# davidepi/glaze

Measured on AMD Instinct MI355X. Metric: Msamples/s + achieved HBM GB/s, Sponza 1080p, 1/2/4/8xMI355X, higher is better.
Workload: dtype f32; 1 GPU; Sponza-class synthetic atrium (262267 tris, 26 materials, 27 textures) as a .glaze V1 file (2853389 bytes) through parse, 1920x1080, path tracer depth 8, 143 steps = 17.9 spp; materials=26, textures=27, scene=Sponza-class synthetic atrium, width=1920, height=1080, depth=8, triangles=262267

## Files before the change

glaze_amd/csrc/abi.cpp:

```cpp
#include <cstring>
#include <string>
#include <vector>

#include "abi_internal.h"
#include "serializer.h"
#include "converter.h"
#include "codec/jpeg.h"
#include "codec/png_enc.h"
#include <strings.h>
#include "rccl_dl.h"

using namespace glz;
using namespace glz::abi;

namespace {
thread_local std::string g_error;
thread_local int g_status = GLZ_OK;

template <class T>
int64_t copy_out(const std::vector<T>& v, T* out, int64_t cap) {
  if (out && cap > 0) memcpy(out, v.data(), sizeof(T) * (size_t)std::min<int64_t>(cap, (int64_t)v.size()));
  return (int64_t)v.size();
}
}
// ... 265 lines not shown
  Renderer* r = Renderer::create(inst->i.get(), scene ? scene->s : std::shared_ptr<Scene>(), w, h, e);
  if (!r) {
    fail(e);
    return nullptr;
  }
  glz_renderer* hr = new glz_renderer();
  hr->r.reset(r);
  return hr;
  GLZ_GUARD_END(nullptr)
}
void glz_renderer_destroy(glz_renderer* h) { delete h; }



int glz_renderer_set_integrator(glz_renderer* h, int i) { GLZ_GUARD_BEGIN GLZ_R(h); GLZ_RET(h->r->set_integrator(i, e)); GLZ_GUARD_END(GLZ_E_IO) }
int glz_renderer_set_exposure(glz_renderer* h, float x) { GLZ_GUARD_BEGIN GLZ_R(h); GLZ_RET(h->r->set_exposure(x)); GLZ_GUARD_END(GLZ_E_IO) }
int glz_renderer_update_camera(glz_renderer* h, const glz_camera* c) {
  GLZ_GUARD_BEGIN GLZ_R(h);
  if (!c) return fail(GLZ_E_ARG, "camera is null");
  GLZ_RET(h->r->update_camera(*c, e));
  GLZ_GUARD_END(GLZ_E_IO)
}
int glz_renderer_change_resolution(glz_renderer* h, uint32_t w, uint32_t hh) { GLZ_GUARD_BEGIN GLZ_R(h); GLZ_RET(h->r->change_resolution(w, hh, e)); GLZ_GUARD_END(GLZ_E_IO) }
int glz_renderer_change_scene(glz_renderer* h, glz_scene* s) {
  GLZ_GUARD_BEGIN GLZ_R(h);
  if (!s || !s->s || !s->owned) return fail(GLZ_E_ARG, "scene is null or already owned by a renderer");
  s->owned = false;
  GLZ_RET(h->r->change_scene(s->s, e));
  GLZ_GUARD_END(GLZ_E_IO)
}
int glz_renderer_update_materials_and_lights(glz_renderer* h, const glz_material* m, uint32_t nm, const glz_light* l, uint32_t nl,
// ... 190 lines not shown
```

glaze_amd/csrc/device/path_state.h:

```cpp
#pragma once
#include <hip/hip_runtime.h>

#include "device/intersect.h"
#include "device/math.h"
#include "device/trace_wave.h"
#include "kernels.h"

namespace glz {
using namespace dev;

constexpr uint32_t kQueueShards = 8;
constexpr uint32_t kCounterStride = 32;
constexpr uint32_t kFlagUpdate = 1u;
constexpr uint32_t kFlagShadow = 2u;

struct PixelId {
  uint32_t x, y;
  bool active;
};
__device__ __forceinline__ PixelId pixel_of(const TileMap& m, uint32_t lid) {
  const uint32_t lane = lid & 63u, sub = (lid >> 6) & 63u, ltile = lid >> 12;
  const uint32_t gtile = ltile * m.world + m.rank;
  const uint32_t tx = gtile % m.tiles_x, ty = gtile / m.tiles_x;
  PixelId p;
// ... 42 lines not shown
      origin = mk3(ro.x, ro.y, ro.z);
      direction = mk3(rd.x, rd.y, rd.z);
    }
    tmin = 0.0001f;
    tmax = INFINITY;
    return true;
  }
};
struct ClosestSink {
  const LaunchArgs& A;
  __device__ __forceinline__ void store(uint32_t lid, const HitRecord& h) {
    A.st.hit[lid] = make_float4(h.leaf == 0xFFFFFFFFu ? INFINITY : h.t, h.u, h.v, __uint_as_float(h.leaf));
  }
};

__device__ __forceinline__ void accumulate_pixel(const LaunchArgs& A, uint32_t lid, vec3 c, bool add, bool update, float exposure, float4 cum) {
  cum.w += 1.0f;
  if (update) {
    if (add) { cum.x += c.x; cum.y += c.y; cum.z += c.z; }
    A.st.result[lid] = make_float4(cum.x * exposure / cum.w, cum.y * exposure / cum.w, cum.z * exposure / cum.w, 1.0f);
  }
  A.st.cumulative[lid] = cum;
}
__device__ __forceinline__ void accumulate_pixel(const LaunchArgs& A, uint32_t lid, vec3 c, bool add, bool update, float exposure) {
  accumulate_pixel(A, lid, c, add, update, exposure, A.st.cumulative[lid]);
}

__device__ __forceinline__ uint32_t queue_capacity(uint32_t n_local_pixels) {
  const uint32_t blocks = (n_local_pixels + kBlock - 1) / kBlock;
  return ((blocks + kQueueShards - 1) / kQueueShards) * kBlock;
}
__device__ __forceinline__ uint32_t queue_slot(uint32_t* counters, uint32_t n_local_pixels, bool push) {
  const unsigned long long m = __ballot(push);
  uint32_t slot = 0;
  if (push) {
    const uint32_t shard = ((blockIdx.x * blockDim.x + threadIdx.x) / kBlock) % kQueueShards;
    const int lane = threadIdx.x & 63;
    const int leader = __ffsll((long long)m) - 1;
    uint32_t base = 0;
    if (lane == leader) base = atomicAdd(counters + shard * kCounterStride, (uint32_t)__popcll(m));
// ... 18 lines not shown
    contrib = A.st.contrib[q];
    lid = __float_as_uint(sd.w);
    o = mk3(so.x, so.y, so.z);
    d = mk3(sd.x, sd.y, sd.z);
    tmin = 0.001f;
    tmax = so.w;
    return true;
  }
};
struct ShadowSink {
  const LaunchArgs& A;
  ShadowSource& src;
  __device__ __forceinline__ void store(uint32_t, const HitRecord& h) {
    const bool occluded = h.leaf != 0xFFFFFFFFu;
    const vec3 c = mk3(src.contrib.x, src.contrib.y, src.contrib.z);
    const bool add = !occluded;
    accumulate_pixel(A, src.lid, c, add, true, A.shadow_exposure);
  }
};
}
```

glaze_amd/csrc/device/shade_pixel.h:

```cpp
#pragma once
#include <hip/hip_runtime.h>

#include "device/hit_vertex.h"
#include "device/math.h"
#include "device/path_state.h"
#include "device/shading.h"
#include "device/types.h"
#include "kernels.h"

namespace glz {
using namespace dev;

struct SharedQueue {
  const LaunchArgs& A;
  __device__ __forceinline__ uint32_t slot(bool push) { return queue_slot(A.st.queue_count + A.shade_set * kQueueSetWords, A.map.n_local_pixels, push); }
};
#ifdef GLZ_SECTION_TIMES
#define GLZ_SHADE_STAMP(k) out.stamp(k)
#else
#define GLZ_SHADE_STAMP(k) do { } while (0)
#endif
struct DirectState {
  const LaunchArgs& A;
  __device__ __forceinline__ void stamp(int) {}
  __device__ __forceinline__ void ray_o(uint32_t lid, float4 v) { A.st.ray_o[lid] = v; }
  __device__ __forceinline__ void ray_d(uint32_t lid, float4 v) { A.st.ray_d[lid] = v; }
  __device__ __forceinline__ void imp(int q, uint32_t lid, float4 v) { A.st.imp[q][lid] = v; }
  __device__ __forceinline__ float4 read_imp(int q, uint32_t lid) const { return A.st.imp[q][lid]; }
  __device__ __forceinline__ void accumulate(uint32_t lid, vec3 c, bool add, bool update, float exposure) { accumulate_pixel(A, lid, c, add && isfinite(c.x + c.y + c.z), update, exposure); }
};
struct StagedState {
#ifdef GLZ_SECTION_TIMES
  unsigned long long sec[8] = {0, 0, 0, 0, 0, 0, 0, 0}, sec_last = 0;
  __device__ __forceinline__ void stamp(int k) {
    const unsigned long long now = __builtin_amdgcn_s_memtime();
    sec[k] += now - sec_last;
    sec_last = now;
  }
#else
  __device__ __forceinline__ void stamp(int) {}
#endif
  float4 ro, rd, im[4];
  uint32_t mask = 0;
  __device__ __forceinline__ void ray_o(uint32_t, float4 v) { ro = v; mask |= 1u; }
  __device__ __forceinline__ void ray_d(uint32_t, float4 v) { rd = v; mask |= 2u; }
  __device__ __forceinline__ void imp(int q, uint32_t, float4 v) { im[q] = v; mask |= 4u; }
  const LaunchArgs* A = nullptr;
  LdsNodePtr lds_imp = nullptr;
  static constexpr uint32_t kShadeBlockPixels = 256;
  __device__ __forceinline__ float4 read_imp(int q, uint32_t) const {
    const u32x4 v = lds_imp[q * kShadeBlockPixels];
    return make_float4(__uint_as_float(v.x), __uint_as_float(v.y), __uint_as_float(v.z), __uint_as_float(v.w));
  }
  __device__ __forceinline__ void accumulate(uint32_t lid, vec3 cc, bool add, bool update, float exposure) { accumulate_pixel(*A, lid, cc, add && isfinite(cc.x + cc.y + cc.z), update, exposure); }
};
template <bool LOD, class Queue, class State>
__device__ __forceinline__ int shade_pixel_body(const LaunchArgs& A, const DeviceScene& S, const FrameData& F, uint32_t lid, PixelId px, float4 ro, float4 rd, float4 hr, Queue& queue,
                                                State& out, float& end_w) {
  const bool fresh = F.direct_only || ro.w == 0.0f;
  float bounce = F.direct_only ? 0.0f : ro.w;
  const vec3 direction = mk3(rd.x, rd.y, rd.z);
  auto load_importance = [&]() {
    asm volatile("" ::: "memory");
    Spec imp;
    if (fresh) {
      imp = spec_set(1.0f);
    } else {
#pragma unroll
      for (int q = 0; q < 4; ++q) {
// ... 2 lines not shown
      }
    }
    return imp;
  };
  const uint32_t leaf = __float_as_uint(hr.w);
  if (leaf == 0xFFFFFFFFu) {
    uint32_t flags = 0;
    vec3 c = mk3(0.0f, 0.0f, 0.0f);
    if ((bounce == 0.0f || rd.w == 1.0f) && S.sky.tex_id > 0) {
      const vec3 w = normalize3(xform_dir(S.sky.world2obj, direction));
      const float phi = glz_atan2f(w.y, w.x), theta = glz_acosf(w.z);
      const vec3 texel = texture_rgb(S, S.sky.tex_id, vec2{phi * kInv2Pi, theta * kInvPi});
      c = spec_to_rgb(spec_mul(load_importance(), from_illuminant_color(texel)));
      flags = kFlagUpdate;
    }
    out.accumulate(lid, c, true, flags != 0, F.exposure);
    end_w = rd.w;
    return F.direct_only ? 0 : 1;
  }
  HitVertex hv = load_hit_vertex(S, hr, [&]() { return A.st.hit_inst[lid]; });
  const MatScalars mat = hv.mat;
  GLZ_SHADE_STAMP(0);
  TexFootprint fp{kNoLod, 0.0f, 0.0f, 1u};
  float cone_w = 0.0f;
  if constexpr (LOD) {
    const auto& [va0, va1, vb0, vb1, vc0, vc1, dn, du_rec] = hv.rec;
    float cone_in = F.cone_width0;
    asm volatile("" : "+v"(cone_in));
    if (!fresh) cone_in = A.st.cone[lid];
    cone_w = cone_in + F.cone_spread * hr.x;
    vec3 e1 = mk3(vb0.x, vb0.y, vb0.z) - mk3(va0.x, va0.y, va0.z), e2 = mk3(vc0.x, vc0.y, vc0.z) - mk3(va0.x, va0.y, va0.z);
// ... 79 lines not shown
      }
    }
    if (!(flags & kFlagShadow)) {
      const Spec importance = load_importance();
      imp_lum = spec_luminance(importance);
      have_lum = true;
    }
    const bool push = (flags & kFlagShadow) != 0;
    GLZ_SHADE_STAMP(3);
    const uint32_t slot = queue.slot(push);
    if (push) {
      A.st.sh_o[slot] = make_float4(point.x, point.y, point.z, sh_tmax);
      A.st.sh_d[slot] = make_float4(sh_dir.x, sh_dir.y, sh_dir.z, __uint_as_float(lid));
      A.st.contrib[slot] = make_float4(c.x, c.y, c.z, __uint_as_float(flags));
    } else {
      out.accumulate(lid, c, true, true, F.exposure);
    }
    spec_flag = 0.0f;
  } else {
    out.accumulate(lid, mk3(0.0f, 0.0f, 0.0f), false, false, F.exposure);
    spec_flag = 1.0f;
  }
  if (F.direct_only) return 0;
  GLZ_SHADE_STAMP(4);
  float rr_scale = 1.0f;
  if (bounce > (float)(F.pt_steps / 2u)) {
    const float kill = gl_max(0.05f, 1.0f - (have_lum ? imp_lum : spec_luminance(load_importance())));
    if (rand01(rng) < kill) {
      end_w = spec_flag;
      return 2;
    }
    rr_scale = 1.0f / (1.0f - kill);
  }
  vec3 xi;
  xi.x = rand01(rng); xi.y = rand01(rng); xi.z = rand01(rng);
// ... 53 lines not shown
```

glaze_amd/csrc/device/types.h:

```cpp
#pragma once
#include <hip/hip_runtime.h>
#include <stdint.h>

namespace glz {

struct Spectrum16 {
  float w[16];
};

struct FrameData {
  uint32_t seed;
  uint32_t lights_no;
  float pixel_offset[2];
  float scene_radius;
  float exposure;
  float scene_size[2];
  float scene_centre[4];
  uint32_t camera_persp;
  uint32_t pt_steps;
  uint32_t direct_only;
  uint32_t lod_mode;
  float cone_spread;
  float cone_width0;
  float next_pixel_offset[2];
  uint32_t pregen;
};

struct RTInstance {
  uint32_t index_offset;
  uint32_t index_count;
// ... 172 lines not shown
```

glaze_amd/csrc/kernels.h:

```cpp
#pragma once
#include <hip/hip_runtime.h>
#include <stdint.h>

#include "device/types.h"
#include "glaze_abi.h"
#include "device_buffer.h"
#include "reproject.h"

namespace glz {

hipError_t launch_derivatives(hipStream_t st, const float4* vertices, const uint32_t* indices, uint32_t n_tris, float4* out);

struct HierarchyInputs {
  const float4* vertices;
  const uint32_t* indices;
  const RTInstance* instances;
  const uint32_t* inst_base;
  uint32_t n_instances;
  const TransformPair* transforms;
  const RTMaterial* materials;
  uint32_t n_world;
  int builder;
  float pair_area_ratio;
  const float4* given_lo = nullptr;
// ... 62 lines not shown
struct TraceCounters {
  unsigned long long closest_rays, shadow_rays, closest_nodes, closest_tris, shadow_nodes, shadow_tris, hits, fresh;
  unsigned long long phase[12];
  unsigned long long shade_tex[4], trace_tex[4];
};

struct LaunchArgs {
  DeviceScene scene;
  PathState st;
  TileMap map;
  FrameData frame;
  CameraConsts cam;
  TraceCounters* counters;
  uint32_t do_closest, do_shadow;
  uint32_t shade_set;
  float shadow_exposure;
};
constexpr uint32_t kPathMaxLaunches = 192;
struct PathBatch {
  uint32_t n;
  uint32_t tables_in_lds;
  uint32_t parity;
  uint32_t seed[kPathMaxLaunches];
  float offset[kPathMaxLaunches + 1][2];
  float exposure[kPathMaxLaunches];
};
constexpr uint32_t kTraceBlock = 256;
constexpr uint32_t kQueueSetWords = 8 * 32;

uint32_t trace_grid_blocks(uint32_t n_local_pixels, bool counting, bool two_level, bool wide8 = false);
hipError_t launch_trace(hipStream_t st, const LaunchArgs& a, uint32_t blocks, bool wide8 = false);
hipError_t launch_shade(hipStream_t st, const LaunchArgs& a);
uint32_t path_grid_blocks(uint32_t n_local_pixels, const DeviceScene& scene);
uint32_t path_resident_blocks(const DeviceScene& scene);
hipError_t launch_path(hipStream_t st, const LaunchArgs& a, const PathBatch& batch, uint32_t blocks);
hipError_t launch_export(hipStream_t st, const TileMap& map, const float4* tiled, float4* frame, bool zero_first);
hipError_t launch_pack_tiles(hipStream_t st, uint32_t n_chain_pixels, uint32_t n_chains, uint32_t chain, const float4* tiled, float4* packed);
hipError_t launch_tonemap(hipStream_t st, uint32_t n_pixels, const float4* result_frame, const float* thresholds, uchar4* out);

uint32_t first_hit_grid_blocks(uint32_t n_rays);
hipError_t launch_first_hit(hipStream_t st, const LaunchArgs& a, uint32_t blocks, float4* hit, uint32_t* inst);
hipError_t launch_first_hit_attributes(hipStream_t st, const LaunchArgs& a, const float4* hit, const uint32_t* inst, float4* aov0, float4* aov1);
constexpr uint32_t kGuideCountWords = GLZ_GUIDE_MAX_BOUNCES + 2;
struct GuideLists {
  float4* o[2];
  float4* d[2];
  uint32_t* count;
};
uint32_t guide_grid_blocks(uint32_t n_rays, uint32_t first_hit_blocks);
hipError_t launch_guide_chain(hipStream_t st, const LaunchArgs& a, uint32_t blocks, uint32_t max_bounces, uint32_t last_list, float4* hit, uint32_t* inst,
// ... 32 lines not shown
```

glaze_amd/csrc/kernels_path.hip:

```cpp
#include "device/path_state.h"
#include "device/shade_pixel.h"
#include "device/trace_wave.h"
#include "launch_geometry.h"

namespace glz {
using namespace dev;

__device__ __forceinline__ void wave_handover_fence() {
  __builtin_amdgcn_fence(__ATOMIC_RELEASE, "wavefront");
  __builtin_amdgcn_fence(__ATOMIC_ACQUIRE, "wavefront");
}

struct GroupHitSink {
  float4* hit;
  __device__ __forceinline__ void store(uint32_t i, const HitRecord& h) {
    hit[i] = make_float4(h.leaf == 0xFFFFFFFFu ? INFINITY : h.t, h.u, h.v, __uint_as_float(h.leaf));
  }
};
struct GroupQueue {
  uint32_t base;
  bool pushed;
  __device__ __forceinline__ uint32_t slot(bool push) {
    const unsigned long long m = __ballot(push);
    pushed = push;
// ... 10 lines not shown
    const uint32_t q = base + i;
    const float4 so = A.st.sh_o[q], sd = A.st.sh_d[q];
    contrib = A.st.contrib[q];
    lid = __float_as_uint(sd.w);
    cum = A.st.cumulative[lid];
    o = mk3(so.x, so.y, so.z);
    d = mk3(sd.x, sd.y, sd.z);
    tmin = 0.001f;
    tmax = so.w;
    return true;
  }
};
struct GroupShadowSink {
  const LaunchArgs& A;
  GroupShadowSource& src;
  float exposure;
  __device__ __forceinline__ void store(uint32_t, const HitRecord& h) {
    const bool occluded = h.leaf != 0xFFFFFFFFu;
    const vec3 c = mk3(src.contrib.x, src.contrib.y, src.contrib.z);
    const bool add = !occluded;
    accumulate_pixel(A, src.lid, c, add, true, exposure, src.cum);
  }
};

struct GroupMixedSource {
  ClosestSource closest;
  GroupShadowSource shadow;
  bool any;
  __device__ __forceinline__ bool load(uint32_t i, vec3& o, vec3& d, float& tmin, float& tmax) {
    any = i >= 64u;
    return any ? shadow.load(i - 64u, o, d, tmin, tmax) : closest.load(i, o, d, tmin, tmax);
  }
};
struct GroupMixedSink {
  GroupHitSink closest;
  GroupShadowSink shadow;
  __device__ __forceinline__ void store(uint32_t i, const HitRecord& h) {
    if (i >= 64u) shadow.store(i - 64u, h); else closest.store(i, h);
  }
};

__device__ __forceinline__ FrameData launch_frame(const LaunchArgs& A, const PathBatch& B, uint32_t L) {
  FrameData F = A.frame;
  F.seed = B.seed[L];
  F.pixel_offset[0] = B.offset[L][0];
  F.pixel_offset[1] = B.offset[L][1];
  F.next_pixel_offset[0] = B.offset[L + 1][0];
  F.next_pixel_offset[1] = B.offset[L + 1][1];
  F.exposure = B.exposure[L];
  return F;
}
constexpr uint32_t kPathBatchOffset = (uint32_t)(((sizeof(LaunchArgs) + alignof(PathBatch) - 1) / alignof(PathBatch)) * alignof(PathBatch));
template <bool LOD>
__device__ __forceinline__ uint32_t path_shade(uint32_t g, uint32_t n_groups, uint32_t lane, uint32_t L, const DeviceScene& S_lds, const float4* hit) {
  const uint32_t lid0 = g * 64u;
  const LaunchArgs& A = *(const LaunchArgs*)reread_kernarg();
  DeviceScene S = A.scene;
  S.tex_counter = nullptr;
  S.srgb_lut = S_lds.srgb_lut;
  S.materials = S_lds.materials;
  S.lights = S_lds.lights;
  S.tex_desc = S_lds.tex_desc;
  const FrameData F = launch_frame(A, *(const PathBatch*)(reread_kernarg() + kPathBatchOffset), L);
  const uint32_t lid = g * 64u + lane;
// ... 51 lines not shown
    const uint32_t lid0 = g * 64u;
    const unsigned long long group_begin = wall_clock64();
    {
      const uint32_t* acc = A.st.path_cost + 4u * (B.parity ^ 1u);
      const unsigned long long sum = (unsigned long long)acc[0] | ((unsigned long long)acc[1] << 32);
      const uint32_t cnt = acc[2], mine = A.st.path_cost[8u + g];
      int prio = 0;
      if (cnt != 0u && mine != 0u) {
        const float r = (float)mine * (float)cnt / (float)sum;
        prio = r > 1.2f ? 3 : (r > 1.08f ? 2 : (r > 0.97f ? 1 : 0));
      }
      prio = __builtin_amdgcn_readfirstlane(prio);
      if (prio == 3) __builtin_amdgcn_s_setprio(3); else if (prio == 2) __builtin_amdgcn_s_setprio(2); else if (prio == 1) __builtin_amdgcn_s_setprio(1); else __builtin_amdgcn_s_setprio(0);
    }
    uint32_t n_shadow = 0;
    float queued_exposure = 0.0f;
    for (uint32_t L = 0;; ++L) {
      const LaunchArgs& A = *(const LaunchArgs*)reread_kernarg();
      const PathBatch& B = *(const PathBatch*)(reread_kernarg() + kPathBatchOffset);
      if (n_shadow != 0u && L == B.n) {
      } else if (L >= B.n) {
        break;
      }
#ifdef GLZ_PATH_TIMES
      const unsigned long long pt0 = wall_clock64();
#endif
      wave_handover_fence();
      if (L < B.n) {
        const FrameData F = launch_frame(A, B, L);
        GroupMixedSource src{ClosestSource{A, F, tally, lid0}, GroupShadowSource{A, lid0, 0u, make_float4(0.0f, 0.0f, 0.0f, 0.0f), make_float4(0.0f, 0.0f, 0.0f, 0.0f)}, false};
        GroupMixedSink sink{GroupHitSink{hit}, GroupShadowSink{A, src.shadow, queued_exposure}};
        trace_wave<false, false, true, GLZ_PATH_PREFETCH != 0>(A.scene, src, sink, &s_stack[threadIdx.x], aux, links, (LdsNodePtr)s_top, A.st.overflow, A.st.overflow_depth, 64u + n_shadow, 0u, 1u, tally);
        n_shadow = 0u;
      } else {
        GroupShadowSource src{A, lid0, 0u, make_float4(0.0f, 0.0f, 0.0f, 0.0f), make_float4(0.0f, 0.0f, 0.0f, 0.0f)};
        GroupShadowSink sink{A, src, queued_exposure};
        trace_wave<true, false, false, GLZ_PATH_PREFETCH != 0>(A.scene, src, sink, &s_stack[threadIdx.x], aux, links, (LdsNodePtr)s_top, A.st.overflow, A.st.overflow_depth, n_shadow, 0u, 1u, tally);
        n_shadow = 0u;
      }
#ifdef GLZ_PATH_TIMES
      const unsigned long long pt1 = wall_clock64();
      pt_trace += pt1 - pt0;
#endif
      wave_handover_fence();
      if (L >= B.n) break;
      n_shadow = path_shade<LOD>(g, n_groups, lane, L, S, hit);
      queued_exposure = B.exposure[L];
#ifdef GLZ_PATH_TIMES
      pt_shade += wall_clock64() - pt1;
#endif
    }
    if (lane == 0u && B.n != 0u) {
      const uint32_t ticks = (uint32_t)((wall_clock64() - group_begin) / B.n);
      A.st.path_cost[8u + g] = ticks;
      uint32_t* acc = A.st.path_cost + 4u * B.parity;
      atomicAdd(reinterpret_cast<unsigned long long*>(acc), (unsigned long long)ticks);
      atomicAdd(acc + 2, 1u);
    }
  }
#ifdef GLZ_PATH_TIMES
  if ((threadIdx.x & 63) == 0 && wave_index() < 8192u) {
    g_path_times[3 * wave_index()] = pt_trace;
// ... 47 lines not shown
```

glaze_amd/csrc/kernels_render.hip:

```cpp
#include "device/path_state.h"
#include "device/shade_pixel.h"
#include "device/trace_wave.h"
#include "device/trace_wave_tl.h"
#include "launch_geometry.h"

namespace glz {
using namespace dev;

constexpr uint32_t kSkyLdsFloats = 1088;
constexpr uint32_t kShadeLdsTableBytes = 8192;

constexpr uint32_t kShadeBlock = 256, kShadeWavesPerBlock = kShadeBlock / 64;
#ifdef GLZ_SECTION_TIMES
static __device__ unsigned long long g_shade_sections[16 * 4096];
#endif
__host__ __device__ inline uint32_t shade_table_quads(const DeviceScene& s) {
  return s.n_materials * (uint32_t)(sizeof(RTMaterial) / 16) + s.n_rt_lights * (uint32_t)(sizeof(RTLight) / 16) + s.n_textures * (uint32_t)(sizeof(TexDesc) / 16);
}
__host__ __device__ inline bool shade_tables_fit(const DeviceScene& s) { return shade_table_quads(s) * 16u <= kShadeLdsTableBytes; }
__host__ __device__ inline bool shade_sky_fits(const DeviceScene& s) { return s.sky_header.marginal_cdf_count > 1u && s.sky_header.marginal_cdf_count <= kSkyLdsFloats; }
template <class T>
__device__ __forceinline__ const T* in_memory(const T* p) { return (const T*)(const __attribute__((address_space(1))) T*)p; }
template <bool COUNT, bool LOD, bool TABLES, bool SKY>
__global__ void __launch_bounds__(kShadeBlock, GLZ_SHADE_WAVES) k_shade(const LaunchArgs A) {
// ... 297 lines not shown
    uint32_t start[kQueueShards + 1];
    start[0] = 0;
#pragma unroll
    for (uint32_t k = 0; k < kQueueShards; ++k) start[k + 1] = start[k] + counts[k * kCounterStride];
    ShadowSource src{A, start, queue_capacity(A.map.n_local_pixels), 0u, make_float4(0.0f, 0.0f, 0.0f, 0.0f)};
    ShadowSink sink{A, src};
    const uint32_t n_waves = wave_count();
    const uint32_t closest_groups = A.do_closest ? (A.map.n_local_pixels + 63u) / 64u : 0u;
    const uint32_t wave = (wave_index() + n_waves - closest_groups % n_waves) % n_waves;
    TraceTally tally;
    trace_wave_tl<true, COUNT>(A.scene, src, sink, &s_stack[threadIdx.x], aux, links, &s_top_ray[threadIdx.x], (LdsNodePtr)s_top, A.st.overflow, A.st.overflow_depth, start[kQueueShards], wave, n_waves, tally);
    if (COUNT) flush_counters(A.counters, true, tally);
  }
}

__global__ void __launch_bounds__(kBlock) k_export(const TileMap map, const float4* __restrict__ tiled, float4* __restrict__ frame) {
  const uint32_t lid = blockIdx.x * kBlock + threadIdx.x;
  const PixelId px = pixel_of(map, lid);
  if (px.active) frame[(size_t)px.y * map.width + px.x] = tiled[lid];
}

__global__ void __launch_bounds__(kBlock) k_pack_tiles(uint32_t n_pixels, uint32_t S, uint32_t s, const float4* __restrict__ chain, float4* __restrict__ packed) {
  const uint32_t i = blockIdx.x * kBlock + threadIdx.x;
  if (i >= n_pixels) return;
  const uint32_t jl = i >> 12, k = i & 4095u;
  packed[(size_t)(jl * S + s) * 4096u + k] = chain[i];
}

__device__ __forceinline__ unsigned char srgb8(const float* __restrict__ thr, float c) {
  if (!(c > 0.0f)) return 0;
// ... 37 lines not shown
  else hipLaunchKernelGGL((k_trace<false, kAlphaNone>), dim3(blocks), dim3(kBlock), 0, st, a);
  return hipGetLastError();
}
hipError_t launch_shade(hipStream_t st, const LaunchArgs& a) {
  if (a.map.n_local_pixels == 0) return hipSuccess;
  const dim3 grid((a.map.n_local_pixels + kShadeBlock - 1) / kShadeBlock), block(kShadeBlock);
  const int which = (a.counters ? 8 : 0) | (a.frame.lod_mode != 0u ? 4 : 0) | (shade_tables_fit(a.scene) ? 2 : 0) | (shade_sky_fits(a.scene) ? 1 : 0);
  switch (which) {
#define GLZ_SHADE_CASE(k) case k: hipLaunchKernelGGL((k_shade<((k) & 8) != 0, ((k) & 4) != 0, ((k) & 2) != 0, ((k) & 1) != 0>), grid, block, 0, st, a); break;
    GLZ_SHADE_CASE(0) GLZ_SHADE_CASE(1) GLZ_SHADE_CASE(2) GLZ_SHADE_CASE(3) GLZ_SHADE_CASE(4) GLZ_SHADE_CASE(5) GLZ_SHADE_CASE(6) GLZ_SHADE_CASE(7)
    GLZ_SHADE_CASE(8) GLZ_SHADE_CASE(9) GLZ_SHADE_CASE(10) GLZ_SHADE_CASE(11) GLZ_SHADE_CASE(12) GLZ_SHADE_CASE(13) GLZ_SHADE_CASE(14) GLZ_SHADE_CASE(15)
#undef GLZ_SHADE_CASE
  }
  return hipGetLastError();
}
hipError_t launch_export(hipStream_t st, const TileMap& map, const float4* tiled, float4* frame, bool zero_first) {
  if (zero_first) {
    hipError_t e = hipMemsetAsync(frame, 0, sizeof(float4) * (size_t)map.width * map.height, st);
    if (e != hipSuccess) return e;
  }
  return launch_per_item(st, k_export, map.n_local_pixels, map, tiled, frame);
}
hipError_t launch_pack_tiles(hipStream_t st, uint32_t n_chain_pixels, uint32_t n_chains, uint32_t chain, const float4* tiled, float4* packed) {
  return launch_per_item(st, k_pack_tiles, n_chain_pixels, n_chain_pixels, n_chains, chain, tiled, packed);
}
hipError_t launch_tonemap(hipStream_t st, uint32_t n, const float4* result_frame, const float* thresholds, uchar4* out) {
  static_assert(kBlock == 256, "k_tonemap stages the 256 thresholds with one load per thread");
  hipLaunchKernelGGL(k_tonemap, grid_for(n), dim3(kBlock), 0, st, n, result_frame, thresholds, out);
  return hipGetLastError();
}
// ... 40 lines not shown
```

glaze_amd/csrc/renderer.cpp:

```cpp
#include "renderer.h"

#include <algorithm>
#include <cmath>
#include <cstdlib>
#include <cstring>

namespace glz {

namespace {
inline bool timed_launch(uint64_t i , uint64_t stride) {
  const uint64_t group = (i - 1) / stride;
  uint32_t x = (uint32_t)group * 747796405u + 2891336453u;
  x = ((x >> ((x >> 28) + 4u)) ^ x) * 277803737u;
  x ^= x >> 22;
  return (i - 1) % stride == x % stride;
}
}
uint64_t Renderer::event_stride() const {
  uint64_t pixels = 0;
  for (const auto& c : chains_) pixels += c->map.n_local_pixels;
  return pixels >= (1u << 20) ? 4u : 16u;
}

Renderer* Renderer::create(Instance* inst, std::shared_ptr<Scene> scene, uint32_t w, uint32_t h, Error& err) {
// ... 114 lines not shown
    const size_t bytes = sizeof(float4) * (size_t)c.map.n_local_pixels;
    DeviceBuffer<float4>* zero[] = {&c.ray_o, &c.ray_d, &c.imp[0], &c.imp[1], &c.imp[2], &c.imp[3], &c.cumulative, &c.result, &c.contrib};
    for (auto* b : zero)
      if (bytes && !hip_ok(hipMemsetAsync(b->ptr, 0, bytes, c.stream), "clear path state", err)) return false;
    if (!hip_ok(hipMemsetAsync(c.queue_count.ptr, 0, sizeof(uint32_t) * 2 * kQueueSetWords, c.stream), "clear queue counters", err)) return false;
    c.shadow_pending = false;
    c.trace_ms = c.shade_ms = c.flush_ms = c.path_ms = 0;
    for (auto& s : c.pending_events) c.free_events.push_back(s);
    c.pending_events.clear();
  }
  if (!hip_ok(hipMemsetAsync(counters_.ptr, 0, sizeof(TraceCounters), chains_[0]->stream), "clear counters", err)) return false;
  if (chains_.size() > 1 && !hip_ok(hipStreamSynchronize(chains_[0]->stream), "clear counters", err)) return false;
  sched_.rewind();
  rng_.reseed(cfg_.seed);
  launches_ = 0;
  request_new_frame_ = false;
  return true;
}

void Renderer::fill_args(const Chain& c, LaunchArgs& a) const {
  a.scene = scene_->dev;
  a.st.ray_o = c.ray_o.ptr;
  a.st.ray_d = c.ray_d.ptr;
  for (int q = 0; q < 4; ++q) a.st.imp[q] = c.imp[q].ptr;
  a.st.hit = c.hit.ptr;
  a.st.cone = c.cone.ptr;
  a.st.hit_inst = c.hit_inst.ptr;
  a.st.sh_o = c.sh_o.ptr;
  a.st.sh_d = c.sh_d.ptr;
  a.st.contrib = c.contrib.ptr;
  a.st.queue_count = c.queue_count.ptr;
  a.st.cumulative = c.cumulative.ptr;
  a.st.result = c.result.ptr;
  a.st.overflow = c.overflow.ptr;
  a.st.overflow_depth = scene_->stack_overflow_depth;
  a.st.path_cost = c.path_cost.ptr;
  a.map = c.map;
  a.cam = cfg_.cam;
  a.counters = cfg_.counting ? counters_.ptr : nullptr;
  a.do_closest = a.do_shadow = 0;
  a.shade_set = c.pending_set ^ 1u;
  a.shadow_exposure = c.pending_exposure;
}

void Renderer::resolve_events(Chain& c) {
  for (auto& s : c.pending_events) {
    float a = 0, b = 0;
    (void)hipEventElapsedTime(&a, s.e[0], s.e[1]);
    if (s.kind == 1) {
      c.flush_ms += a;
    } else if (s.kind == 2) {
      c.path_ms += a;
    } else {
      (void)hipEventElapsedTime(&b, s.e[1], s.e[2]);
      const double weight = (double)s.weight;
      c.trace_ms += a * weight;
      c.shade_ms += b * weight;
// ... 43 lines not shown
    c.pending_events.push_back(ev);
  }
};

bool Renderer::flush_shadows(Chain& c, Error& err) {
  if (!c.shadow_pending) return true;
  LaunchArgs a;
  fill_args(c, a);
  memset(&a.frame, 0, sizeof(a.frame));
  a.do_shadow = 1;
  Timed t{c};
  if (!t.begin(*this, cfg_.profile_kernels, 1, 0, err)) return false;
  if (!hip_ok(launch_trace(c.stream, a, trace_grid(c), wide8()), "k_trace (shadow pass)", err)) return false;
  t.end();
  c.shadow_pending = false;
  return true;
}

bool Renderer::launch_constants_common(FrameData& fd, Error& err) {
  if (request_new_frame_ && !reset_buffers(err)) return false;
  memset(&fd, 0, sizeof(fd));
  fd.lights_no = scene_->lights_no;
  fd.scene_radius = scene_->data.meta.scene_radius;
  fd.scene_size[0] = (float)w_;
  fd.scene_size[1] = (float)h_;
  for (int k = 0; k < 3; ++k) fd.scene_centre[k] = scene_->data.meta.scene_centre[k];
  fd.camera_persp = cfg_.camera.type == GLZ_CAMERA_PERSPECTIVE ? 1u : 0u;
  fd.pt_steps = cfg_.pt_steps;
  fd.direct_only = cfg_.integrator == GLZ_DIRECT ? 1u : 0u;
  fd.lod_mode = (uint32_t)cfg_.lod_mode;
// ... 2 lines not shown
    const bool persp = cfg_.camera.type == GLZ_CAMERA_PERSPECTIVE;
    fd.cone_spread = persp ? pixel : 0.0f;
    fd.cone_width0 = persp ? 0.0f : pixel;
    if (!scene_->mips_ready() && !scene_->ensure_mips(err)) return false;
  }
  fd.pregen = fd.direct_only ? 0u : 1u;
  return true;
}

bool Renderer::one_launch(Error& err) {
  FrameData fd;
  if (!launch_constants_common(fd, err)) return false;
  fd.seed = rng_.next();
  sched_.next(fd.pixel_offset);
  sched_.peek(fd.next_pixel_offset);
  fd.exposure = cfg_.exposure;
  ++launches_;
  if (fd.lights_no == 0) return true;
  for (auto& cp : chains_) {
    Chain& c = *cp;
    hipStream_t st = c.stream;
    LaunchArgs a;
    fill_args(c, a);
    a.frame = fd;
    a.do_closest = 1;
    a.do_shadow = c.shadow_pending ? 1u : 0u;
    const uint64_t stride = event_stride();
    Timed t{c};
    if (!t.begin(*this, cfg_.profile_kernels && timed_launch(launches_, stride), 0, (uint32_t)stride, err)) return false;
    if (!hip_ok(launch_trace(st, a, trace_grid(c), wide8()), "k_trace", err)) return false;
    t.mark();
    if (!hip_ok(launch_shade(st, a), "k_shade", err)) return false;
    t.end();
    c.shadow_pending = true;
    c.pending_set = a.shade_set;
    c.pending_exposure = cfg_.exposure;
  }
  return true;
}

bool Renderer::path_batch(uint32_t n, Error& err) {
  FrameData fd;
  if (!launch_constants_common(fd, err)) return false;
  PathBatch b;
  memset(&b, 0, sizeof(b));
  b.n = n;
  b.parity = chains_[0]->path_batches++ & 1u;
  for (uint32_t i = 0; i < n; ++i) {
    b.seed[i] = rng_.next();
    sched_.next(b.offset[i]);
    b.exposure[i] = cfg_.exposure;
  }
  sched_.peek(b.offset[n]);
  launches_ += n;
  if (fd.lights_no == 0) return true;
  Chain& c = *chains_[0];
  if (!flush_shadows(c, err)) return false;
  LaunchArgs a;
  fill_args(c, a);
  a.frame = fd;
  a.counters = nullptr;
  Timed t{c};
  if (!t.begin(*this, cfg_.profile_kernels, 2, 0, err)) return false;
  if (!hip_ok(hipMemsetAsync(c.path_cost.ptr + 4u * b.parity, 0, 16, c.stream), "clear path cost accumulator", err)) return false;
  if (!hip_ok(launch_path(c.stream, a, b, c.grid_path), "k_path", err)) return false;
  t.end();
  return true;
}

bool Renderer::run_launches(uint32_t n, Error& err) {
// ... 87 lines not shown
}

bool Renderer::set_integrator(int integrator, Error& err) {
  if (integrator != GLZ_DIRECT && integrator != GLZ_PATH_TRACE) {
    err.code = GLZ_E_ARG;
    err.msg = "unknown integrator";
    return false;
  }
  if (integrator != cfg_.integrator) {
    cfg_.integrator = integrator;
    request_new_frame_ = true;
  }
  return group_.forward([=](Renderer& p, Error& e) { return p.set_integrator(integrator, e); }, err);
}

bool Renderer::set_exposure(float e) {
  if (e >= 0.0f) cfg_.exposure = e;
  group_.each([=](Renderer& p) { p.set_exposure(e); });
  return true;
}

bool Renderer::update_camera(const glz_camera& c, Error& err) {
  if (c.type > GLZ_CAMERA_ORTHOGRAPHIC) {
    err.code = GLZ_E_ARG;
    err.msg = "unknown camera type";
    return false;
  }
  cfg_.camera = c;
  host::push_constants(cfg_.camera, w_, h_, cfg_.cam.camera2world, cfg_.cam.screen2camera);
  request_new_frame_ = true;
  const glz_camera cam = c;
  return group_.forward([=](Renderer& p, Error& e) { return p.update_camera(cam, e); }, err);
}

// ... 106 lines not shown
}

bool Renderer::gather(bool result, float4* dst, Error& err, bool zero_first) {
  if (!settle(err)) return false;
  hipStream_t st = chains_[0]->stream;
  bool first = zero_first;
  for (auto& c : chains_) {
    if (!hip_ok(launch_export(st, c->map, result ? c->result.ptr : c->cumulative.ptr, dst, first), "k_export", err)) return false;
    first = false;
  }
  return group_.empty() || group_.bring_tiles(result, dst, err);
}

bool Renderer::settle(Error& err) {
  if (request_new_frame_ && !reset_buffers(err)) return false;
  return wait_idle(err);
}

bool Renderer::to_host(std::initializer_list<HostCopy> copies, const char* what, Error& err) const {
  hipStream_t st = inst_->stream;
  for (const HostCopy& c : copies)
    if (!hip_ok(hipMemcpyAsync(c.out, c.dev, c.bytes, hipMemcpyDeviceToHost, st), what, err)) return false;
  return hip_ok(hipStreamSynchronize(st), what, err);
}
bool Renderer::rgba8_to_host(const float4* frame, uint8_t* out, const char* what, const char* what_sync, Error& err) {
  hipStream_t st = chains_[0]->stream;
  if (!hip_ok(launch_tonemap(st, w_ * h_, frame, oetf_thresholds_.ptr, rgba8_.ptr), "k_tonemap", err)) return false;
  if (!hip_ok(hipMemcpyAsync(out, rgba8_.ptr, (size_t)w_ * h_ * 4, hipMemcpyDeviceToHost, st), what, err)) return false;
  return hip_ok(hipStreamSynchronize(st), what_sync, err);
}
// ... 191 lines not shown
```

glaze_amd/csrc/renderer.h:

```cpp
#pragma once
#include <cstdlib>
#include <initializer_list>
#include <memory>
#include <vector>

#include "device_group.h"
#include "host_math.h"
#include "kernels.h"
#include "post_stage.h"
#include "scene.h"
#include "tile_map.h"

namespace glz {

class Renderer {
 public:
  static Renderer* create(Instance* inst, std::shared_ptr<Scene> scene , uint32_t w, uint32_t h, Error& err);
  ~Renderer();

  bool set_integrator(int integrator, Error& err);
  bool set_exposure(float e);
  bool update_camera(const glz_camera& c, Error& err);
  bool change_resolution(uint32_t w, uint32_t h, Error& err);
  bool change_scene(std::shared_ptr<Scene> scene, Error& err);
  bool update_materials_and_lights(const glz_material* m, uint32_t nm, const glz_light* l, uint32_t nl, const glz_texture* t, uint32_t nt, Error& err);
  bool refresh_binded_textures(const glz_texture* t, uint32_t nt, Error& err);
  bool update_transforms(const glz_transform* t, uint32_t n, Error& err);
  bool wait_idle(Error& err);
  uint32_t steps_per_sample() const { return cfg_.integrator == GLZ_DIRECT ? 1u : cfg_.pt_steps; }

  bool draw(size_t spp, void (*cb)(void*), void* user, uint8_t* rgba8_out, Error& err);
  bool restart();
  bool step(uint32_t n, Error& err);
  bool read_rgba8(uint8_t* out, Error& err);
  bool read_frame(bool result, float* out, Error& err);
  PostStage& post() { return post_; }
// ... 97 lines not shown
  uint64_t event_stride() const;
  struct Chain {
    TileMap map{};
    hipStream_t stream = nullptr;
    bool own_stream = false;
    DeviceBuffer<float4> ray_o, ray_d, imp[4], hit, sh_o, sh_d, contrib, cumulative, result;
    DeviceBuffer<float> cone;
    DeviceBuffer<uint32_t> hit_inst;
    DeviceBuffer<uint32_t> overflow, queue_count, path_cost;
    uint32_t path_batches = 0;
    uint32_t grid = 0, grid_counting = 0;
    uint32_t grid8 = 0;
    uint32_t grid_path = 0;
    bool shadow_pending = false;
    uint32_t pending_set = 0;
    float pending_exposure = 1.0f;
    std::vector<EventSet> pending_events;
    std::vector<EventSet> free_events;
    double trace_ms = 0, shade_ms = 0, flush_ms = 0, path_ms = 0;
  };
  std::vector<std::unique_ptr<Chain>> chains_;
  uint32_t pick_chains() const;
  uint32_t trace_grid(const Chain& c) const { return cfg_.counting ? c.grid_counting : (wide8() ? c.grid8 : c.grid); }
  void release_chains();
  bool flush_shadows(Chain& c, Error& err);
  bool acquire_events(Chain& c, EventSet& ev, Error& err);
  void resolve_events(Chain& c);
  void fill_args(const Chain& c, LaunchArgs& a) const;

  DeviceGroup group_{*this};
  bool wait_idle_local(const char* what, Error& err);
  bool step_local(uint32_t n, Error& err);

  bool frame_is_here(const char* who, Error& err) const;
  bool read_post(bool filter, float* rgba32f, uint8_t* rgba8, Error& err, hipEvent_t* marks = nullptr);
  PostStage post_{*this};

  DeviceBuffer<float4> frame_tmp_;
  DeviceBuffer<uchar4> rgba8_;
  DeviceBuffer<float> oetf_thresholds_;
  DeviceBuffer<TraceCounters> counters_;
  uint64_t launches_ = 0;
};

}
```

Before: 2843 Msamples/s.

## Defer per-sample result normalization to a finalize kernel using launch-ordinal marks

Per-sample accumulation no longer writes the normalized result buffer or increments a sample count. Each pixel now stores a negative launch ordinal as a marker in cumulative.w, and pixels that receive no contribution skip the cumulative write entirely. A new finalize kernel, run at settle time or on an exposure change, computes result = sum*exposure/count for the marked pixels and restores the count. This cuts per-bounce HBM read/write traffic, in exchange for an extra resolve pass and tighter coupling between host-side launch counting and the device-side marks.

```diff
diff --git a/glaze_amd/csrc/abi.cpp b/glaze_amd/csrc/abi.cpp
--- a/glaze_amd/csrc/abi.cpp
+++ b/glaze_amd/csrc/abi.cpp
@@ -303,7 +303,7 @@
 
 
 int glz_renderer_set_integrator(glz_renderer* h, int i) { GLZ_GUARD_BEGIN GLZ_R(h); GLZ_RET(h->r->set_integrator(i, e)); GLZ_GUARD_END(GLZ_E_IO) }
-int glz_renderer_set_exposure(glz_renderer* h, float x) { GLZ_GUARD_BEGIN GLZ_R(h); GLZ_RET(h->r->set_exposure(x)); GLZ_GUARD_END(GLZ_E_IO) }
+int glz_renderer_set_exposure(glz_renderer* h, float x) { GLZ_GUARD_BEGIN GLZ_R(h); GLZ_RET(h->r->set_exposure(x, e)); GLZ_GUARD_END(GLZ_E_IO) }
 int glz_renderer_update_camera(glz_renderer* h, const glz_camera* c) {
   GLZ_GUARD_BEGIN GLZ_R(h);
   if (!c) return fail(GLZ_E_ARG, "camera is null");
diff --git a/glaze_amd/csrc/device/path_state.h b/glaze_amd/csrc/device/path_state.h
--- a/glaze_amd/csrc/device/path_state.h
+++ b/glaze_amd/csrc/device/path_state.h
@@ -80,16 +80,15 @@
   }
 };
 
-__device__ __forceinline__ void accumulate_pixel(const LaunchArgs& A, uint32_t lid, vec3 c, bool add, bool update, float exposure, float4 cum) {
-  cum.w += 1.0f;
-  if (update) {
-    if (add) { cum.x += c.x; cum.y += c.y; cum.z += c.z; }
-    A.st.result[lid] = make_float4(cum.x * exposure / cum.w, cum.y * exposure / cum.w, cum.z * exposure / cum.w, 1.0f);
-  }
-  A.st.cumulative[lid] = cum;
+__device__ __forceinline__ float update_mark(uint32_t ordinal) { return -(float)(ordinal < (1u << 24) ? ordinal : (1u << 24)); }
+__device__ __forceinline__ void accumulate_retired(const LaunchArgs& A, uint32_t lid, vec3 c, bool add, float mark, float4 cum) {
+  if (add) A.st.cumulative[lid] = make_float4(cum.x + c.x, cum.y + c.y, cum.z + c.z, mark);
+  else A.st.cumulative[lid].w = mark;
 }
-__device__ __forceinline__ void accumulate_pixel(const LaunchArgs& A, uint32_t lid, vec3 c, bool add, bool update, float exposure) {
-  accumulate_pixel(A, lid, c, add, update, exposure, A.st.cumulative[lid]);
+__device__ __forceinline__ void accumulate_shaded(const LaunchArgs& A, uint32_t lid, vec3 c, bool add, bool update, float mark) {
+  if (!update) return;
+  const float4 cum = A.st.cumulative[lid];
+  A.st.cumulative[lid] = make_float4(add ? cum.x + c.x : cum.x, add ? cum.y + c.y : cum.y, add ? cum.z + c.z : cum.z, mark);
 }
 
 __device__ __forceinline__ uint32_t queue_capacity(uint32_t n_local_pixels) {
@@ -138,8 +137,8 @@
   __device__ __forceinline__ void store(uint32_t, const HitRecord& h) {
     const bool occluded = h.leaf != 0xFFFFFFFFu;
     const vec3 c = mk3(src.contrib.x, src.contrib.y, src.contrib.z);
-    const bool add = !occluded;
-    accumulate_pixel(A, src.lid, c, add, true, A.shadow_exposure);
+    if (occluded) A.st.cumulative[src.lid].w = A.shadow_mark;
+    else accumulate_retired(A, src.lid, c, true, A.shadow_mark, A.st.cumulative[src.lid]);
   }
 };
 }
diff --git a/glaze_amd/csrc/device/shade_pixel.h b/glaze_amd/csrc/device/shade_pixel.h
--- a/glaze_amd/csrc/device/shade_pixel.h
+++ b/glaze_amd/csrc/device/shade_pixel.h
@@ -27,7 +27,7 @@
   __device__ __forceinline__ void ray_d(uint32_t lid, float4 v) { A.st.ray_d[lid] = v; }
   __device__ __forceinline__ void imp(int q, uint32_t lid, float4 v) { A.st.imp[q][lid] = v; }
   __device__ __forceinline__ float4 read_imp(int q, uint32_t lid) const { return A.st.imp[q][lid]; }
-  __device__ __forceinline__ void accumulate(uint32_t lid, vec3 c, bool add, bool update, float exposure) { accumulate_pixel(A, lid, c, add && isfinite(c.x + c.y + c.z), update, exposure); }
+  __device__ __forceinline__ void accumulate(uint32_t lid, vec3 c, bool add, bool update, float mark) { accumulate_shaded(A, lid, c, add && isfinite(c.x + c.y + c.z), update, mark); }
 };
 struct StagedState {
 #ifdef GLZ_SECTION_TIMES
@@ -52,7 +52,7 @@
     const u32x4 v = lds_imp[q * kShadeBlockPixels];
     return make_float4(__uint_as_float(v.x), __uint_as_float(v.y), __uint_as_float(v.z), __uint_as_float(v.w));
   }
-  __device__ __forceinline__ void accumulate(uint32_t lid, vec3 cc, bool add, bool update, float exposure) { accumulate_pixel(*A, lid, cc, add && isfinite(cc.x + cc.y + cc.z), update, exposure); }
+  __device__ __forceinline__ void accumulate(uint32_t lid, vec3 cc, bool add, bool update, float mark) { accumulate_shaded(*A, lid, cc, add && isfinite(cc.x + cc.y + cc.z), update, mark); }
 };
 template <bool LOD, class Queue, class State>
 __device__ __forceinline__ int shade_pixel_body(const LaunchArgs& A, const DeviceScene& S, const FrameData& F, uint32_t lid, PixelId px, float4 ro, float4 rd, float4 hr, Queue& queue,
@@ -85,7 +85,7 @@
       c = spec_to_rgb(spec_mul(load_importance(), from_illuminant_color(texel)));
       flags = kFlagUpdate;
     }
-    out.accumulate(lid, c, true, flags != 0, F.exposure);
+    if (flags != 0) out.accumulate(lid, c, true, true, F.update_mark);
     end_w = rd.w;
     return F.direct_only ? 0 : 1;
   }
@@ -195,11 +195,10 @@
       A.st.sh_d[slot] = make_float4(sh_dir.x, sh_dir.y, sh_dir.z, __uint_as_float(lid));
       A.st.contrib[slot] = make_float4(c.x, c.y, c.z, __uint_as_float(flags));
     } else {
-      out.accumulate(lid, c, true, true, F.exposure);
+      out.accumulate(lid, c, true, true, F.update_mark);
     }
     spec_flag = 0.0f;
   } else {
-    out.accumulate(lid, mk3(0.0f, 0.0f, 0.0f), false, false, F.exposure);
     spec_flag = 1.0f;
   }
   if (F.direct_only) return 0;
diff --git a/glaze_amd/csrc/device/types.h b/glaze_amd/csrc/device/types.h
--- a/glaze_amd/csrc/device/types.h
+++ b/glaze_amd/csrc/device/types.h
@@ -13,7 +13,7 @@
   uint32_t lights_no;
   float pixel_offset[2];
   float scene_radius;
-  float exposure;
+  float update_mark;
   float scene_size[2];
   float scene_centre[4];
   uint32_t camera_persp;
diff --git a/glaze_amd/csrc/kernels.h b/glaze_amd/csrc/kernels.h
--- a/glaze_amd/csrc/kernels.h
+++ b/glaze_amd/csrc/kernels.h
@@ -100,7 +100,7 @@
   TraceCounters* counters;
   uint32_t do_closest, do_shadow;
   uint32_t shade_set;
-  float shadow_exposure;
+  float shadow_mark;
 };
 constexpr uint32_t kPathMaxLaunches = 192;
 struct PathBatch {
@@ -109,7 +109,7 @@
   uint32_t parity;
   uint32_t seed[kPathMaxLaunches];
   float offset[kPathMaxLaunches + 1][2];
-  float exposure[kPathMaxLaunches];
+  uint32_t base_ordinal;
 };
 constexpr uint32_t kTraceBlock = 256;
 constexpr uint32_t kQueueSetWords = 8 * 32;
@@ -120,6 +120,7 @@
 uint32_t path_grid_blocks(uint32_t n_local_pixels, const DeviceScene& scene);
 uint32_t path_resident_blocks(const DeviceScene& scene);
 hipError_t launch_path(hipStream_t st, const LaunchArgs& a, const PathBatch& batch, uint32_t blocks);
+hipError_t launch_finalize(hipStream_t st, const TileMap& map, float4* cumulative, float4* result, float exposure, float launches);
 hipError_t launch_export(hipStream_t st, const TileMap& map, const float4* tiled, float4* frame, bool zero_first);
 hipError_t launch_pack_tiles(hipStream_t st, uint32_t n_chain_pixels, uint32_t n_chains, uint32_t chain, const float4* tiled, float4* packed);
 hipError_t launch_tonemap(hipStream_t st, uint32_t n_pixels, const float4* result_frame, const float* thresholds, uchar4* out);
diff --git a/glaze_amd/csrc/kernels_path.hip b/glaze_amd/csrc/kernels_path.hip
--- a/glaze_amd/csrc/kernels_path.hip
+++ b/glaze_amd/csrc/kernels_path.hip
@@ -48,12 +48,12 @@
 struct GroupShadowSink {
   const LaunchArgs& A;
   GroupShadowSource& src;
-  float exposure;
+  float mark;
   __device__ __forceinline__ void store(uint32_t, const HitRecord& h) {
     const bool occluded = h.leaf != 0xFFFFFFFFu;
     const vec3 c = mk3(src.contrib.x, src.contrib.y, src.contrib.z);
     const bool add = !occluded;
-    accumulate_pixel(A, src.lid, c, add, true, exposure, src.cum);
+    accumulate_retired(A, src.lid, c, add, mark, src.cum);
   }
 };
 
@@ -81,7 +81,7 @@
   F.pixel_offset[1] = B.offset[L][1];
   F.next_pixel_offset[0] = B.offset[L + 1][0];
   F.next_pixel_offset[1] = B.offset[L + 1][1];
-  F.exposure = B.exposure[L];
+  F.update_mark = update_mark(B.base_ordinal + L + 1u);
   return F;
 }
 constexpr uint32_t kPathBatchOffset = (uint32_t)(((sizeof(LaunchArgs) + alignof(PathBatch) - 1) / alignof(PathBatch)) * alignof(PathBatch));
@@ -163,7 +163,7 @@
       if (prio == 3) __builtin_amdgcn_s_setprio(3); else if (prio == 2) __builtin_amdgcn_s_setprio(2); else if (prio == 1) __builtin_amdgcn_s_setprio(1); else __builtin_amdgcn_s_setprio(0);
     }
     uint32_t n_shadow = 0;
-    float queued_exposure = 0.0f;
+    float queued_mark = 0.0f;
     for (uint32_t L = 0;; ++L) {
       const LaunchArgs& A = *(const LaunchArgs*)reread_kernarg();
       const PathBatch& B = *(const PathBatch*)(reread_kernarg() + kPathBatchOffset);
@@ -178,12 +178,12 @@
       if (L < B.n) {
         const FrameData F = launch_frame(A, B, L);
         GroupMixedSource src{ClosestSource{A, F, tally, lid0}, GroupShadowSource{A, lid0, 0u, make_float4(0.0f, 0.0f, 0.0f, 0.0f), make_float4(0.0f, 0.0f, 0.0f, 0.0f)}, false};
-        GroupMixedSink sink{GroupHitSink{hit}, GroupShadowSink{A, src.shadow, queued_exposure}};
+        GroupMixedSink sink{GroupHitSink{hit}, GroupShadowSink{A, src.shadow, queued_mark}};
         trace_wave<false, false, true, GLZ_PATH_PREFETCH != 0>(A.scene, src, sink, &s_stack[threadIdx.x], aux, links, (LdsNodePtr)s_top, A.st.overflow, A.st.overflow_depth, 64u + n_shadow, 0u, 1u, tally);
         n_shadow = 0u;
       } else {
         GroupShadowSource src{A, lid0, 0u, make_float4(0.0f, 0.0f, 0.0f, 0.0f), make_float4(0.0f, 0.0f, 0.0f, 0.0f)};
-        GroupShadowSink sink{A, src, queued_exposure};
+        GroupShadowSink sink{A, src, queued_mark};
         trace_wave<true, false, false, GLZ_PATH_PREFETCH != 0>(A.scene, src, sink, &s_stack[threadIdx.x], aux, links, (LdsNodePtr)s_top, A.st.overflow, A.st.overflow_depth, n_shadow, 0u, 1u, tally);
         n_shadow = 0u;
       }
@@ -194,7 +194,7 @@
       wave_handover_fence();
       if (L >= B.n) break;
       n_shadow = path_shade<LOD>(g, n_groups, lane, L, S, hit);
-      queued_exposure = B.exposure[L];
+      queued_mark = update_mark(B.base_ordinal + L + 1u);
 #ifdef GLZ_PATH_TIMES
       pt_shade += wall_clock64() - pt1;
 #endif
diff --git a/glaze_amd/csrc/kernels_render.hip b/glaze_amd/csrc/kernels_render.hip
--- a/glaze_amd/csrc/kernels_render.hip
+++ b/glaze_amd/csrc/kernels_render.hip
@@ -335,6 +335,17 @@
   }
 }
 
+__global__ void __launch_bounds__(kBlock) k_finalize(const TileMap map, float4* __restrict__ cumulative, float4* __restrict__ result, float exposure, float launches) {
+  const uint32_t lid = blockIdx.x * kBlock + threadIdx.x;
+  if (!pixel_of(map, lid).active) return;
+  const float4 cum = cumulative[lid];
+  if (cum.w < 0.0f) {
+    const float w = -cum.w;
+    result[lid] = make_float4(cum.x * exposure / w, cum.y * exposure / w, cum.z * exposure / w, 1.0f);
+  }
+  if (cum.w != launches) cumulative[lid].w = launches;
+}
+
 __global__ void __launch_bounds__(kBlock) k_export(const TileMap map, const float4* __restrict__ tiled, float4* __restrict__ frame) {
   const uint32_t lid = blockIdx.x * kBlock + threadIdx.x;
   const PixelId px = pixel_of(map, lid);
@@ -402,6 +413,9 @@
   }
   return hipGetLastError();
 }
+hipError_t launch_finalize(hipStream_t st, const TileMap& map, float4* cumulative, float4* result, float exposure, float launches) {
+  return launch_per_item(st, k_finalize, map.n_local_pixels, map, cumulative, result, exposure, launches);
+}
 hipError_t launch_export(hipStream_t st, const TileMap& map, const float4* tiled, float4* frame, bool zero_first) {
   if (zero_first) {
     hipError_t e = hipMemsetAsync(frame, 0, sizeof(float4) * (size_t)map.width * map.height, st);
diff --git a/glaze_amd/csrc/renderer.cpp b/glaze_amd/csrc/renderer.cpp
--- a/glaze_amd/csrc/renderer.cpp
+++ b/glaze_amd/csrc/renderer.cpp
@@ -152,6 +152,8 @@
   sched_.rewind();
   rng_.reseed(cfg_.seed);
   launches_ = 0;
+  accum_launches_ = 0;
+  resolve_pending_ = false;
   request_new_frame_ = false;
   return true;
 }
@@ -178,7 +180,7 @@
   a.counters = cfg_.counting ? counters_.ptr : nullptr;
   a.do_closest = a.do_shadow = 0;
   a.shade_set = c.pending_set ^ 1u;
-  a.shadow_exposure = c.pending_exposure;
+  a.shadow_mark = c.pending_mark;
 }
 
 void Renderer::resolve_events(Chain& c) {
@@ -252,6 +254,17 @@
   if (!hip_ok(launch_trace(c.stream, a, trace_grid(c), wide8()), "k_trace (shadow pass)", err)) return false;
   t.end();
   c.shadow_pending = false;
+  return true;
+}
+
+bool Renderer::resolve(Error& err) {
+  if (!resolve_pending_) return true;
+  for (auto& cp : chains_) {
+    Chain& c = *cp;
+    if (!flush_shadows(c, err)) return false;
+    if (!hip_ok(launch_finalize(c.stream, c.map, c.cumulative.ptr, c.result.ptr, cfg_.exposure, -update_mark()), "k_finalize", err)) return false;
+  }
+  resolve_pending_ = false;
   return true;
 }
 
@@ -284,9 +297,11 @@
   fd.seed = rng_.next();
   sched_.next(fd.pixel_offset);
   sched_.peek(fd.next_pixel_offset);
-  fd.exposure = cfg_.exposure;
   ++launches_;
   if (fd.lights_no == 0) return true;
+  ++accum_launches_;
+  resolve_pending_ = true;
+  fd.update_mark = update_mark();
   for (auto& cp : chains_) {
     Chain& c = *cp;
     hipStream_t st = c.stream;
@@ -304,7 +319,7 @@
     t.end();
     c.shadow_pending = true;
     c.pending_set = a.shade_set;
-    c.pending_exposure = cfg_.exposure;
+    c.pending_mark = fd.update_mark;
   }
   return true;
 }
@@ -319,11 +334,13 @@
   for (uint32_t i = 0; i < n; ++i) {
     b.seed[i] = rng_.next();
     sched_.next(b.offset[i]);
-    b.exposure[i] = cfg_.exposure;
   }
   sched_.peek(b.offset[n]);
   launches_ += n;
   if (fd.lights_no == 0) return true;
+  b.base_ordinal = (uint32_t)std::min<uint64_t>(accum_launches_, 1u << 24);
+  accum_launches_ += n;
+  resolve_pending_ = true;
   Chain& c = *chains_[0];
   if (!flush_shadows(c, err)) return false;
   LaunchArgs a;
@@ -441,10 +458,12 @@
   return group_.forward([=](Renderer& p, Error& e) { return p.set_integrator(integrator, e); }, err);
 }
 
-bool Renderer::set_exposure(float e) {
-  if (e >= 0.0f) cfg_.exposure = e;
-  group_.each([=](Renderer& p) { p.set_exposure(e); });
-  return true;
+bool Renderer::set_exposure(float e, Error& err) {
+  if (e >= 0.0f && e != cfg_.exposure) {
+    if (resolve_pending_ && !request_new_frame_ && !(hip_ok(hipSetDevice(inst_->device), "hipSetDevice", err) && resolve(err))) return false;
+    cfg_.exposure = e;
+  }
+  return group_.forward([=](Renderer& p, Error& pe) { return p.set_exposure(e, pe); }, err);
 }
 
 bool Renderer::update_camera(const glz_camera& c, Error& err) {
@@ -581,6 +600,7 @@
 
 bool Renderer::settle(Error& err) {
   if (request_new_frame_ && !reset_buffers(err)) return false;
+  if (!hip_ok(hipSetDevice(inst_->device), "hipSetDevice", err) || !resolve(err)) return false;
   return wait_idle(err);
 }
 
diff --git a/glaze_amd/csrc/renderer.h b/glaze_amd/csrc/renderer.h
--- a/glaze_amd/csrc/renderer.h
+++ b/glaze_amd/csrc/renderer.h
@@ -1,4 +1,5 @@
 #pragma once
+#include <algorithm>
 #include <cstdlib>
 #include <initializer_list>
 #include <memory>
@@ -19,7 +20,7 @@
   ~Renderer();
 
   bool set_integrator(int integrator, Error& err);
-  bool set_exposure(float e);
+  bool set_exposure(float e, Error& err);
   bool update_camera(const glz_camera& c, Error& err);
   bool change_resolution(uint32_t w, uint32_t h, Error& err);
   bool change_scene(std::shared_ptr<Scene> scene, Error& err);
@@ -147,7 +148,7 @@
     uint32_t grid_path = 0;
     bool shadow_pending = false;
     uint32_t pending_set = 0;
-    float pending_exposure = 1.0f;
+    float pending_mark = 0.0f;
     std::vector<EventSet> pending_events;
     std::vector<EventSet> free_events;
     double trace_ms = 0, shade_ms = 0, flush_ms = 0, path_ms = 0;
@@ -157,6 +158,8 @@
   uint32_t trace_grid(const Chain& c) const { return cfg_.counting ? c.grid_counting : (wide8() ? c.grid8 : c.grid); }
   void release_chains();
   bool flush_shadows(Chain& c, Error& err);
+  bool resolve(Error& err);
+  float update_mark() const { return -(float)std::min<uint64_t>(accum_launches_, 1u << 24); }
   bool acquire_events(Chain& c, EventSet& ev, Error& err);
   void resolve_events(Chain& c);
   void fill_args(const Chain& c, LaunchArgs& a) const;
@@ -174,6 +177,8 @@
   DeviceBuffer<float> oetf_thresholds_;
   DeviceBuffer<TraceCounters> counters_;
   uint64_t launches_ = 0;
+  uint64_t accum_launches_ = 0;
+  bool resolve_pending_ = false;
 };
 
 }
```

Measured after the change: 2929 Msamples/s (median of 6 runs). +3.0%, better.
